# wenet-e2e/wetts

Measured on AMD Instinct MI355X. Metric: audio samples/sec + RTF @22.05 kHz, VITS-Baker, 1/2/4/8 MI355X, higher is better.
Workload: dtype f32

## Files before the change

wetts_amd/csrc/common.h:

```cpp
#pragma once
#include <hip/hip_runtime.h>
#include <stdint.h>
#include <stdio.h>
#include <string>

#include <string.h>

#include "../../include/wetts_hip.h"

namespace wetts {

void set_error(const char* fmt, ...);

#define WETTS_HIP_CHECK(expr)                                                        \
  do {                                                                               \
    hipError_t _e = (expr);                                                          \
    if (_e != hipSuccess) {                                                          \
      ::wetts::set_error("%s failed: %s (%s:%d)", #expr, hipGetErrorString(_e),      \
                         __FILE__, __LINE__);                                        \
      return WETTS_E_HIP;                                                            \
    }                                                                                \
  } while (0)

static inline bool lds_opt_in(const void* kernel, signed char* state) {
// ... 89 lines not shown
  int64_t wn_mask_stride;
  int wn_H, wn_last, wn_first;
};

inline ConvParams conv_io(const float* x, int Cin, int T, float* out, int Cout, int B) {
  ConvParams p;
  memset(&p, 0, sizeof(p));
  p.x = x;
  p.x_bs = (int64_t)Cin * T;
  p.x_cs = T;
  p.Tin = T;
  p.in_rev_base = -1;
  p.in_act = IN_NONE;
  p.in_slope = 0.f;
  p.out = out;
  p.o_bs = (int64_t)Cout * T;
  p.o_cs = T;
  p.Tout = T;
  p.out_act = OUT_NONE;
  p.out_div = 1.f;
  p.B = B;
  return p;
}

struct PackedConv {
  float* wpk = nullptr;
  const float* bias = nullptr;
  int M = 0, Cin = 0, ktaps = 0, dil = 1, pad = 0;
  int up = 0, up_pad = 0;
  int Cout = 0;
  int k_orig = 0;
  int off_lo = 0, span = 0, nchunks = 0;
  int gate_H = 0;
};

int32_t pack_conv_weight(const float* w_dev, const float* bias_dev, int Cout, int Cin, int k,
                         int dil, int pad, int transposed, int up, hipStream_t stream,
                         PackedConv* out, int rev_in = 0, int gate_H = 0);
void free_packed(PackedConv* pc);

int32_t launch_conv(const PackedConv& pc, ConvParams p, hipStream_t stream);
bool pw_gemm_eligible(const PackedConv& pc, const ConvParams& p);
int32_t launch_pw_gemm(const PackedConv& pc, const ConvParams& p, hipStream_t stream, int variant);
int32_t launch_conv_group(const PackedConv* const* pcs, const ConvParams* ps, int n, hipStream_t stream,
                          int* launches = nullptr);

int conv_variant();
void set_conv_variant(int v);
int32_t launch_conv_small(const ConvParams& p, hipStream_t stream, bool* taken);
struct SmallConvScope {
  explicit SmallConvScope(int max_tiles);
  ~SmallConvScope();
  int prev;
};

inline int cdiv(int a, int b) { return (a + b - 1) / b; }
inline int64_t align_up(int64_t v, int64_t a) { return (v + a - 1) / a * a; }

inline int device_cus() {
  static int cus = 0;
  if (cus == 0) {
    int dev = 0, n = 0;
    cus = (hipGetDevice(&dev) == hipSuccess &&
           hipDeviceGetAttribute(&n, hipDeviceAttributeMultiprocessorCount, dev) == hipSuccess && n > 0) ? n : 256;
  }
  return cus;
}

}
```

wetts_amd/csrc/conv_mfma.hip:

```cpp
#include <stdlib.h>

#include "common.h"

namespace wetts {

typedef float f32x16 __attribute__((ext_vector_type(16)));
typedef float f32x4v __attribute__((ext_vector_type(4)));
constexpr int kBufRsrcDword3 = 0x00020000;

__device__ __forceinline__ float lrelu2(float x, float slope) {
  const float m = x * slope;
  float r;
  asm("v_max_f32 %0, %1, %2" : "=v"(r) : "v"(x), "v"(m));
  return r;
}

__global__ void pack_conv_weight_kernel(const float* __restrict__ w, float* __restrict__ out,
                                        int M, int Cin, int Cout, int k, int ktaps, int up,
                                        int transposed, int rev_in, int gate_H, int G, int64_t total) {
  int64_t idx = (int64_t)blockIdx.x * blockDim.x + threadIdx.x;
  if (idx >= total) return;
  int s = (int)(idx & 3);
  int lane = (int)((idx >> 2) & 63);
  int64_t rest = idx >> 8;
// ... 36 lines not shown
    pc->dil = dil;
    pc->pad = pad;
    pc->up = 0;
    pc->up_pad = 0;
  } else {
    pc->M = Cout * up;
    pc->ktaps = cdiv(k, up);
    pc->dil = -1;
    pc->pad = 0;
    pc->up = up;
    pc->up_pad = pad;
  }
  int o0 = -pc->pad, o1 = (pc->ktaps - 1) * pc->dil - pc->pad;
  pc->off_lo = o0 < o1 ? o0 : o1;
  pc->span = (o0 < o1 ? o1 : o0) - pc->off_lo;
  pc->nchunks = cdiv(Cin, kConvCK);
  int G = pc->nchunks * pc->ktaps * 2;
  int mt32 = cdiv(pc->M, 128) * 4;
  int64_t total = (int64_t)mt32 * G * 256;
  WETTS_HIP_CHECK(hipMalloc((void**)&pc->wpk, (total + (int64_t)G * 256) * sizeof(float)));
  WETTS_HIP_CHECK(hipMemsetAsync(pc->wpk + total, 0, (size_t)G * 256 * sizeof(float), stream));
  int threads = 256;
  int64_t blocks = (total + threads - 1) / threads;
  hipLaunchKernelGGL(pack_conv_weight_kernel, dim3((unsigned)blocks), dim3(threads), 0, stream,
                     w_dev, pc->wpk, pc->M, Cin, Cout, k, pc->ktaps, up > 0 ? up : 1, transposed,
                     rev_in, gate_H, G, total);
  WETTS_LAUNCH_CHECK();
  return WETTS_OK;
}

void free_packed(PackedConv* pc) {
  if (pc->wpk) (void)hipFree(pc->wpk);
  pc->wpk = nullptr;
}

constexpr int conv_fixed_stride(int nt) { return ((nt + 132 - 32 + 63) / 64) * 64 + 32; }
constexpr bool conv_has_fixed_stride(int nt) { return nt <= 256; }

template <int MB, int NB, int WM, int WN, int EPI, bool FAST>
__device__ __forceinline__ void conv_mfma_body(const ConvParams& p, int bid) {
  static_assert(WM * WN == 4, "4 waves per block");
  constexpr int CK = kConvCK;
  constexpr int MT = 32 * MB * WM;
  constexpr int NT = 32 * NB * WN;
  constexpr int MAXCI = (NT + 128 + 63) / 64;
  constexpr int RPW = CK / 4;

  extern __shared__ __attribute__((aligned(16))) float smem[];

  const int tid = threadIdx.x;
  const int lane = tid & 63;
  const int wave = __builtin_amdgcn_readfirstlane(tid >> 6);
  const int wm = wave / WN, wn = wave % WN;

  const int ntiles = (p.N + NT - 1) / NT;
  const int mtiles = (p.M + MT - 1) / MT;
  const int ntile = bid % ntiles;
  bid /= ntiles;
  const int mtile = bid % mtiles;
  const int b = bid / mtiles;

  const int n0 = ntile * NT;
  int Tin = p.Tin, Tout = p.Tout, N = p.N;
  if (p.lens) {
    Tin = min((int)p.lens[b] * p.len_mul, p.Tin);
    Tout = p.up > 0 ? Tin * p.up : Tin;
// ... 426 lines not shown
        if (omask) v *= omask[t];
        float* dst = p.out + ob + (int64_t)co * p.o_cs + t;
        if (!pre_res) {
          if (p.res) v += p.res[rb + (int64_t)co * p.r_cs + t];
          if (p.accum) v += *dst;
        }
        if (p.out_div != 1.f) v = mrf_div(v, p.out_div, 1.f / p.out_div, mrf_div_fast(p.out_div));
        *dst = v;
      }
    }
  }
}

template <int MB, int NB, int WM, int WN, int EPI = 0, bool MRF = false, bool FAST = false>
__global__ __launch_bounds__(256) __attribute__((amdgpu_waves_per_eu((MB * NB >= 4 && WN < 4) ? 3 : 1)))
void conv_mfma_kernel(const ConvParams p) {
  conv_mfma_body<MB, NB, WM, WN, EPI, FAST>(p, blockIdx.x);
}

constexpr int kConvGroupMax = 3;
struct ConvGroupParams {
  ConvParams p[kConvGroupMax];
  int first[kConvGroupMax + 1];
  int n;
};
template <int MB, int NB, int WM, int WN, int EPI>
__global__ __launch_bounds__(256) __attribute__((amdgpu_waves_per_eu((MB * NB >= 4 && WN < 4) ? 3 : 1)))
void conv_mfma_group_kernel(const ConvGroupParams gp) {
  const int bid = blockIdx.x;
  int j = 0;
  if (gp.n > 1 && bid >= gp.first[1]) j = 1;
  if (gp.n > 2 && bid >= gp.first[2]) j = 2;
  conv_mfma_body<MB, NB, WM, WN, EPI, true>(gp.p[j], bid - gp.first[j]);
}



static bool conv_fast_ok(const ConvParams& p);

static int g_conv_variant = -1;

int conv_variant() {
  if (g_conv_variant < 0) {
    const char* e = getenv("WETTS_CONV_VARIANT");
    g_conv_variant = e ? atoi(e) : 0;
  }
  return g_conv_variant;
}
void set_conv_variant(int v) { g_conv_variant = v; }

template <int MB, int NB, int WM, int WN>
static int32_t launch_cfg(const ConvParams& p, hipStream_t stream) {
  constexpr int MT = 32 * MB * WM, NT = 32 * NB * WN;
  int ntiles = cdiv(p.N, NT), mtiles = cdiv(p.M, MT);
  int64_t blocks = (int64_t)ntiles * mtiles * p.B;
  if (blocks <= 0) return WETTS_OK;
  WETTS_REQUIRE(blocks < (1ll << 31), "conv grid too large");
  const bool fast = conv_fast_ok(p);
  const size_t lds = (size_t)2 * kConvCK *
                     (fast ? (conv_has_fixed_stride(NT) ? conv_fixed_stride(NT) : ((NT + p.span + 3 + 3) & ~3)) : NT + p.span) *
                     sizeof(float);
  const dim3 grid((unsigned)blocks), blk(256);
  const bool plain = p.up == 0 && p.out_act == OUT_NONE && p.out_mask == nullptr && p.wn_skip == nullptr;
  if (p.out_act == OUT_GATE) {
    if (fast)
      hipLaunchKernelGGL((conv_mfma_kernel<MB, NB, WM, WN, 5, false, true>), grid, blk, lds, stream, p);
// ... 43 lines not shown
  p.ktaps = pc.ktaps;
  p.dil = pc.dil;
  p.pad = pc.pad;
  p.off_lo = pc.off_lo;
  p.span = pc.span;
  p.nchunks = pc.nchunks;
  p.up = pc.up;
  p.up_pad = pc.up_pad;
  p.up_shift = -1;
  for (int q = 0; q < 16; ++q)
    if (pc.up == (1 << q)) p.up_shift = q;
  WETTS_REQUIRE(pc.wpk != nullptr, "conv weight not packed");
  WETTS_REQUIRE((p.out_act == OUT_GATE) == (pc.gate_H > 0), "gate epilogue and interleaved packing go together");
  WETTS_REQUIRE(p.out_act != OUT_GATE || (!p.res && !p.accum && !p.out_mask && p.out_div == 1.f && !p.wn_skip && pc.up == 0),
                "gate epilogue: plain store only");
  if (pc.ktaps == 1 && pc.up == 0 && p.in_mask && p.in_mask == p.out_mask &&
      p.in_mask_stride == p.out_mask_stride && p.out_act == OUT_NONE)
    p.in_mask = nullptr;
  WETTS_REQUIRE(p.span <= 128, "conv receptive field too wide (span %d > 128)", p.span);
  if (p.up > 0) {
    p.N = p.Tin + p.ktaps - 1;
  } else {
    p.N = p.Tout;
  }
  return WETTS_OK;
}

static bool conv_fast_ok(const ConvParams& p) {
  return p.in_mask == nullptr && p.in_rev_base < 0 && (p.Cin % kConvCK) == 0 && (p.x_cs & 3) == 0 &&
         (p.x_bs & 3) == 0 && (p.Tin & 3) == 0 && p.span <= 125 && (reinterpret_cast<uintptr_t>(p.x) & 15) == 0 &&
         ((int64_t)p.Cin * p.x_cs) < (1ll << 29) && (p.lens == nullptr || (p.len_mul & 3) == 0);
}

template <int MB, int NB, int WM, int WN>
static int32_t launch_group_cfg(ConvGroupParams& gp, int max_span, hipStream_t stream) {
  constexpr int MT = 32 * MB * WM, NT = 32 * NB * WN;
  int64_t total = 0;
  for (int j = 0; j < gp.n; ++j) {
    gp.first[j] = (int)total;
    total += (int64_t)cdiv(gp.p[j].N, NT) * cdiv(gp.p[j].M, MT) * gp.p[j].B;
  }
  gp.first[gp.n] = (int)total;
  WETTS_REQUIRE(total > 0 && total < (1ll << 31), "conv group grid size");
  const size_t lds = (size_t)2 * kConvCK * (conv_has_fixed_stride(NT) ? conv_fixed_stride(NT) : ((NT + max_span + 3 + 3) & ~3)) *
                     sizeof(float);
  hipLaunchKernelGGL((conv_mfma_group_kernel<MB, NB, WM, WN, 1>), dim3((unsigned)total), dim3(256), lds, stream, gp);
  WETTS_LAUNCH_CHECK();
  return WETTS_OK;
}

int32_t launch_conv_group(const PackedConv* const* pcs, const ConvParams* ps, int n, hipStream_t stream,
                          int* launches) {
  if (launches) *launches = n;
  if (n <= 0) return WETTS_OK;
  ConvGroupParams gp;
  memset(&gp, 0, sizeof(gp));
  bool ok = n >= 2 && n <= kConvGroupMax && conv_variant() == 0;
  int order[kConvGroupMax] = {0, 1, 2};
  if (ok) {
    for (int a = 0; a < n; ++a)
      for (int b = a + 1; b < n; ++b)
        if (pcs[order[b]]->ktaps > pcs[order[a]]->ktaps) { int t = order[a]; order[a] = order[b]; order[b] = t; }
  }
  int max_span = 0;
  for (int j = 0; j < n && ok; ++j) {
    gp.p[j] = ps[order[j]];
    WETTS_TRY(prepare_conv(*pcs[order[j]], gp.p[j]));
    const ConvParams& q = gp.p[j];
    ok = q.up == 0 && q.out_act == OUT_NONE && q.out_mask == nullptr && q.out_div == 1.f && q.tag && conv_fast_ok(q) &&
         q.M == gp.p[0].M && q.N == gp.p[0].N && q.B == gp.p[0].B && q.Cin == gp.p[0].Cin && q.lens == gp.p[0].lens;
    if (q.span > max_span) max_span = q.span;
  }
  gp.n = n;
  if (ok) {
    const ConvParams& q = gp.p[0];
    const int64_t cols = (int64_t)q.N * q.B;
    auto nblk = [&](int mt, int nt) { return (int64_t)cdiv(q.M, mt) * cdiv(q.N, nt) * q.B; };
    if (q.M >= 128 && cols >= 4096 && nblk(128, 128) >= 384) {
      if (launches) *launches = 1;
      return launch_group_cfg<1, 4, 4, 1>(gp, max_span, stream);
    }
    if (q.M > 32 && q.M < 128 && cols >= 8192 && nblk(64, 256) >= 384) {
      if (launches) *launches = 1;
      return launch_group_cfg<1, 4, 2, 2>(gp, max_span, stream);
    }
  }
  for (int j = 0; j < n; ++j) WETTS_TRY(launch_conv(*pcs[j], ps[j], stream));
  return WETTS_OK;
}

int32_t launch_conv(const PackedConv& pc, ConvParams p, hipStream_t stream) {
  WETTS_TRY(prepare_conv(pc, p));
  if (conv_variant() == 0 && p.lens == nullptr) {
    bool taken = false;
    WETTS_TRY(launch_conv_small(p, stream, &taken));
    if (taken) return WETTS_OK;
  }
  {
    const int v = conv_variant();
    if ((v == 0 || (v >= 7 && v <= 9)) && pw_gemm_eligible(pc, p)) return launch_pw_gemm(pc, p, stream, v);
  }
  const int64_t cols = (int64_t)p.N * p.B;
  switch (conv_variant()) {
    case 2: return launch_cfg<1, 2, 4, 1>(p, stream);
    case 3: return launch_cfg<1, 4, 2, 2>(p, stream);
    case 4: return launch_cfg<1, 2, 2, 2>(p, stream);
    case 5: return launch_cfg<1, 1, 2, 2>(p, stream);
    case 6: return launch_cfg<1, 4, 4, 1>(p, stream);
    default: break;
  }
  auto nblk = [&](int mt, int nt) { return (int64_t)cdiv(p.M, mt) * cdiv(p.N, nt) * p.B; };
  constexpr int64_t kFill = 384;
  if (p.M >= 128 && cols >= 4096) {
    const int64_t n128 = nblk(128, 128);
    const int kCUs = device_cus();
    if (n128 >= 4 * kCUs) return launch_cfg<1, 4, 4, 1>(p, stream);
    auto cost = [&](int64_t blocks, int area, double eff) {
      return (blocks < kCUs ? 4.0 : 1.0) * (double)((blocks + kCUs - 1) / kCUs) * area / eff;
    };
    const double c128 = cost(n128, 128 * 128, 1.18), c64w = cost(nblk(64, 128), 64 * 128, 1.07),
                 c64 = cost(nblk(64, 64), 64 * 64, 1.0);
    if (c128 <= c64w && c128 <= c64) return launch_cfg<1, 4, 4, 1>(p, stream);
    if (c64w <= c64) return launch_cfg<1, 2, 2, 2>(p, stream);
    return launch_cfg<1, 1, 2, 2>(p, stream);
  }
// ... 11 lines not shown
```

wetts_amd/csrc/kernels.hip:

```cpp
#include "kernels.h"

namespace wetts {

static inline dim3 grid1d(int64_t n, int threads) {
  return dim3((unsigned)((n + threads - 1) / threads));
}

__global__ void embed_mask_kernel(const int64_t* __restrict__ ids,
                                  const int64_t* __restrict__ lengths,
                                  const float* __restrict__ emb, int n_vocab, int B, int H, int T,
                                  float scale, float* __restrict__ x_out,
                                  float* __restrict__ mask_out, int32_t* __restrict__ status) {
  int64_t idx = (int64_t)blockIdx.x * blockDim.x + threadIdx.x;
  int64_t total = (int64_t)B * H * T;
  if (idx >= total) return;
  int t = (int)(idx % T);
  int c = (int)((idx / T) % H);
  int b = (int)(idx / ((int64_t)T * H));
  bool valid = (int64_t)t < lengths[b];
  float v = 0.f;
  if (valid) {
    int64_t id = ids[(int64_t)b * T + t];
    if (id < 0 || id >= n_vocab) {
      if (status && c == 0) atomicOr(status, WETTS_STATUS_PHONE_ID_RANGE);
// ... 622 lines not shown
#pragma unroll
        for (int i = 0; i < 10; ++i) win[i] = raw[i] > 0.f ? raw[i] : raw[i] * 0.01f;
#pragma unroll
        for (int j = 0; j < 7; ++j) {
          const float wv = wsh[(c + u) * 7 + j];
#pragma unroll
          for (int o = 0; o < 4; ++o) acc[o] += wv * win[o + j];
        }
      }
    }
  } else
  for (int c = 0; c < C; ++c) {
    const float* xr = xb + (int64_t)c * T;
    float win[4 + 15];
    for (int i = 0; i < 3 + k; ++i) {
      int tt = t0 - pad + i;
      float v = (tt >= 0 && tt < Tb) ? xr[tt] : 0.f;
      win[i] = v > 0.f ? v : v * 0.01f;
    }
    for (int j = 0; j < k; ++j) {
      float wv = wsh[c * k + j];
#pragma unroll
      for (int o = 0; o < 4; ++o) acc[o] += wv * win[o + j];
    }
  }
#pragma unroll
  for (int o = 0; o < 4; ++o)
    if (t0 + o < T) out[(int64_t)b * T + t0 + o] = (t0 + o < Tb) ? tanhf(acc[o]) : 0.f;
}

template <int K>
__global__ __launch_bounds__(256) void conv_post_tanh_small_kernel(const float* __restrict__ x,
                                                                   const float* __restrict__ w, int B,
                                                                   int C, int T, float* __restrict__ out) {
  constexpr int TL = 32, CG = 8, MAXC = 8;
  __shared__ float red[CG][TL + 1];
  const int tl = threadIdx.x % TL, cg = threadIdx.x / TL;
  const int tblocks = (T + TL - 1) / TL;
  const int b = blockIdx.x / tblocks;
  const int t = (blockIdx.x % tblocks) * TL + tl;
  constexpr int pad = (K - 1) / 2;
  const float* xb = x + (int64_t)b * C * T;
  float win[MAXC][K], wv[MAXC][K];
#pragma unroll
  for (int j = 0; j < MAXC; ++j) {
    const int c = cg + CG * j;
    const int cc = c < C ? c : 0;
#pragma unroll
    for (int i = 0; i < K; ++i) {
      const int tt = t - pad + i;
      const bool ok = c < C && tt >= 0 && tt < T;
      win[j][i] = xb[(int64_t)cc * T + (ok ? tt : 0)];
      wv[j][i] = ok ? w[cc * K + i] : 0.f;
    }
  }
  float acc = 0.f;
#pragma unroll
  for (int j = 0; j < MAXC; ++j)
#pragma unroll
    for (int i = 0; i < K; ++i) {
      const float v = win[j][i];
      acc += wv[j][i] * (v > 0.f ? v : v * 0.01f);
    }
  red[cg][tl] = acc;
  __syncthreads();
  if (cg == 0 && t < T) {
    float tot = 0.f;
#pragma unroll
    for (int q = 0; q < CG; ++q) tot += red[q][tl];
    out[(int64_t)b * T + t] = tanhf(tot);
  }
}

int32_t k_conv_post_tanh(const float* x, const float* w, int k, int B, int C, int T, float* out,
                         hipStream_t s, const int64_t* lens, int len_mul) {
  WETTS_REQUIRE(k <= 15, "conv_post kernel size %d unsupported", k);
  int64_t n = (int64_t)B * ((T + 3) / 4);
  if (n == 0) return WETTS_OK;
  if (k == 7 && C <= 64 && n <= 64 * 256 && !lens) {
    hipLaunchKernelGGL(conv_post_tanh_small_kernel<7>, dim3((unsigned)(B * cdiv(T, 32))), dim3(256), 0, s, x, w,
                       B, C, T, out);
    WETTS_LAUNCH_CHECK();
    return WETTS_OK;
  }
  hipLaunchKernelGGL(conv_post_tanh_kernel, grid1d(n, 256), dim3(256), (size_t)C * k * 4, s, x, w,
                     k, B, C, T, out, lens, len_mul);
  WETTS_LAUNCH_CHECK();
  return WETTS_OK;
}

__global__ __launch_bounds__(64) void durations_kernel(const float* __restrict__ logw,
                                                       const float* __restrict__ mask,
                                                       float length_scale, int B, int T,
                                                       float* __restrict__ w_ceil,
                                                       float* __restrict__ cum,
                                                       int64_t* __restrict__ y_lengths,
                                                       int32_t* __restrict__ status) {
  const int b = blockIdx.x, lane = threadIdx.x;
  float carry = 0.f;
  for (int t0 = 0; t0 < T; t0 += 64) {
    int t = t0 + lane;
    float wc = 0.f;
    if (t < T) {
      float w = expf(logw[(int64_t)b * T + t]) * mask[(int64_t)b * T + t] * length_scale;
      wc = ceilf(w);
      w_ceil[(int64_t)b * T + t] = wc;
    }
    float v = wc;
#pragma unroll
    for (int off = 1; off < 64; off <<= 1) {
      float n = __shfl_up(v, off, 64);
      if (lane >= off) v += n;
    }
    v += carry;
// ... 564 lines not shown
```

wetts_amd/csrc/model.hip:

```cpp
#include <stdarg.h>
#include <stdlib.h>
#include <string.h>

#include <map>
#include <string>
#include <vector>

#include "common.h"
#include "conv_bf16.h"
#include "resblock32.h"
#include "qconv_u8.h"
#include "kernels.h"

namespace wetts {

static thread_local char g_err[512] = "";

void set_error(const char* fmt, ...) {
  va_list ap;
  va_start(ap, fmt);
  vsnprintf(g_err, sizeof(g_err), fmt, ap);
  va_end(ap);
}

// ... 366 lines not shown
  int fuse32_maxc = 32;
  int fuse32_kmax = 99;
  int fuse32_kwide = 3;
  int fuse2_maxc = 128;
  int fuse_min_blocks = 128;
  int small_max_tiles = 256;
  int chain_whole_waste_pct = 15;
  int chain_whole_maxc = 64;
  int chain_pair_maxc = 32;
  int chain_pair_kmax = 3;
  int fuse2_waste_pct = 20;
  mutable int flow_precision = 0;
  mutable std::vector<std::vector<PackedConvB>> b_wn_in, b_wn_rs;
  mutable PackedConvB b_post;
  mutable float* b_post_wpad = nullptr;
  mutable PackedQConv q_pre, q_cond, q_post;
  mutable std::vector<std::vector<PackedQConv>> q_c1, q_c2;
  mutable bool q_packed = false;
  mutable int flow_packed_prec = 0, dec_packed_prec = 0;
  mutable std::vector<PackedConvB> b_ups;
  mutable PackedConvB b_pre;
  mutable std::vector<std::vector<PackedConvB>> b_c1, b_c2;
  mutable int32_t* status_word = nullptr;
  mutable uint64_t rng_seed = 0, rng_offset = 0;
  int mrf_streams = 1;
  int mrf_fork_maxc = 1 << 20;
  int stage2_pct = 30;
  int dds_fused = 1;
  int attn_small_max_t = 128;
  int wn_gate = 1;
  int wn_fuse = 1;
  int small_fork = 1;
  int conv_groups = 1;
  hipStream_t aux_stream[WETTS_MAX_RB_KERNELS] = {};
  hipEvent_t ev_fork = nullptr, ev_chain[WETTS_MAX_RB_KERNELS] = {};
  bool fork_ok = false;

  int spec_channels = 0;
  bool post_loaded = false;
  Layout post_layout;
  float* post_blob = nullptr;
  PackedConv pe_pre, pe_proj;
  std::vector<PackedConv> pe_in, pe_rs, fwd_pre;
  const float *pe_cond_w = nullptr, *pe_cond_b = nullptr;

  bool dur_loaded = false;
  Layout dur_layout;
  float* dur_blob = nullptr;
  ConvFlowW dur_cf1;
  std::vector<ConvFlowW> dur_post_cf;
  const float *dur_post_pre_w = nullptr, *dur_post_pre_b = nullptr;
  PackedConv dur_post_proj;
  DDS dur_post_dds;
  const float *dur_qm = nullptr, *dur_qlogs = nullptr;

  const float* T(const std::string& name) const { return tensor(layout, blob, name); }
};

namespace wetts {

struct Bump {
  char* base;
  int64_t cap, off = 0;
  bool ok = true;
  Bump(void* p, int64_t c) : base((char*)p), cap(c) {}
  template <typename T>
// ... 481 lines not shown
  return L.total;
}

int32_t wetts_create(const wetts_config_t* cfg, const float* blob_dev, int64_t blob_numel,
                     void* stream, wetts_model_t** out) {
  WETTS_TRY(validate_config(cfg));
  WETTS_REQUIRE(out != nullptr && blob_dev != nullptr, "null argument");
  hipStream_t s = (hipStream_t)stream;
  wetts_model* m = new wetts_model();
  m->cfg = *cfg;
  build_layout(cfg, m->layout);
  if (blob_numel != m->layout.total) {
    set_error("blob has %lld floats, layout needs %lld", (long long)blob_numel,
              (long long)m->layout.total);
    delete m;
    return WETTS_E_INVALID;
  }
  hipError_t e = hipMalloc((void**)&m->blob, (size_t)blob_numel * sizeof(float));
  if (e != hipSuccess) {
    set_error("hipMalloc(blob) failed: %s", hipGetErrorString(e));
    delete m;
    return WETTS_E_HIP;
  }
  e = hipMemcpyAsync(m->blob, blob_dev, (size_t)blob_numel * sizeof(float),
                     hipMemcpyDeviceToDevice, s);
  int32_t r = (e == hipSuccess) ? build_model(m, s) : WETTS_E_HIP;
  {
    struct Knob { const char* name; int* field; };
    const Knob knobs[] = {
        {"stage2_pct", &m->stage2_pct}, {"dds_fused", &m->dds_fused}, {"wn_fuse", &m->wn_fuse}, {"wn_gate", &m->wn_gate},
        {"fuse2_waste_pct", &m->fuse2_waste_pct}, {"fuse_min_blocks", &m->fuse_min_blocks},
        {"chain_whole_pct", &m->chain_whole_waste_pct}, {"chain_whole_maxc", &m->chain_whole_maxc},
        {"small_max_tiles", &m->small_max_tiles}, {"attn_small_max_t", &m->attn_small_max_t},
    };
    if (const char* env = getenv("WETTS_TUNE")) {
      std::string all(env);
      size_t pos = 0;
      while (pos < all.size()) {
        size_t end = all.find(',', pos);
        if (end == std::string::npos) end = all.size();
        const std::string item = all.substr(pos, end - pos);
        const size_t eq = item.find('=');
        bool known = false;
        if (eq != std::string::npos)
          for (const Knob& k : knobs)
            if (item.compare(0, eq, k.name) == 0 && strlen(k.name) == eq) {
              *k.field = atoi(item.c_str() + eq + 1);
              known = true;
            }
        if (!known && !item.empty()) {
          set_error("WETTS_TUNE: unknown setting '%s'", item.c_str());
          r = WETTS_E_INVALID;
        }
        pos = end + 1;
      }
    }
    if (r == WETTS_OK && !m->wn_gate) {
      for (int f = 0; f < cfg->flow_n_flows && r == WETTS_OK; ++f)
        for (int i = 0; i < cfg->flow_wn_layers && r == WETTS_OK; ++i) {
          free_packed(&m->flows[f].in_layers[i]);
          r = pack(m->layout, m->blob, S("flow.flows.%d.enc.in_layers.%d", flow_key_stride(cfg) * f, i), s,
                   &m->flows[f].in_layers[i]);
        }
    }
    if (m->mrf_streams < 1) m->mrf_streams = 1;
    if (m->mrf_streams > cfg->n_resblock_kernels) m->mrf_streams = cfg->n_resblock_kernels;
    m->fork_ok = hipEventCreateWithFlags(&m->ev_fork, hipEventDisableTiming) == hipSuccess && m->ev_fork;
    for (int j = 0; j < cfg->n_resblock_kernels; ++j) {
      if (hipEventCreateWithFlags(&m->ev_chain[j], hipEventDisableTiming) != hipSuccess || !m->ev_chain[j]) m->fork_ok = false;
      if (j > 0)
        if (hipStreamCreateWithFlags(&m->aux_stream[j], hipStreamNonBlocking) != hipSuccess || !m->aux_stream[j]) m->fork_ok = false;
    }
    (void)hipGetLastError();
  }
  if (r == WETTS_OK) {
    e = hipStreamSynchronize(s);
    if (e != hipSuccess) {
      set_error("weight packing failed: %s", hipGetErrorString(e));
      r = WETTS_E_HIP;
    }
  }
  if (r != WETTS_OK) {
    wetts_destroy(m);
    return r;
  }
  *out = m;
  return WETTS_OK;
}

void wetts_destroy(wetts_model_t* m) {
  if (!m) return;
  free_posterior(m);
  free_duration(m);
  for (PackedConv* pc : m->all_packed) free_packed(pc);
  for (auto& pc : m->b_ups) free_packed_bf16(&pc);
  for (auto& v : m->b_c1) for (auto& pc : v) free_packed_bf16(&pc);
// ... 1223 lines not shown
        p2.r_bs = (int64_t)ch * len;
        p2.r_cs = len;
        p2.accum = accum;
        p2.out_div = odiv;
        p2.tag = 1;
        p2.lens = lens;
        p2.len_mul = spf;
        if (last_d || m->dec_unfused) {
          WETTS_TRY(launch_conv(rb.c2[d], p2, s));
          count(1, 3 + accum);
        } else {
          g2[n2] = &rb.c2[d];
          p2s[n2++] = p2;
        }
      }
      rx[j] = outp[j];
    }
    if (n2 > 0) {
      int nl = 0;
      WETTS_TRY(launch_conv_group(g2, p2s, n2, s, &nl));
      count(nl, 3.0 * n2);
    }
  }
  return WETTS_OK;
}

static int32_t run_hifigan(const wetts_model* m, const float* z, int64_t z_bs, int64_t z_cs,
                           const float* y_mask, int64_t mask_stride, const float* g, int B, int L,
                           float* audio, void* workspace, int64_t workspace_bytes, hipStream_t s,
                           DecTiming* tm, const int64_t* lens = nullptr) {
  const wetts_config_t* c = &m->cfg;
  const int I = c->inter_channels, C0 = c->upsample_initial_channel;
  const int64_t mx = dec_max_elems(c, B, L);
  Bump ws(workspace, workspace_bytes);
  float* bx = ws.take<float>(mx);
  float* bt = ws.take<float>(mx);
  float* bs = ws.take<float>(mx);
  float* chain_buf[WETTS_MAX_RB_KERNELS][3];
  for (int j = 0; j < c->n_resblock_kernels; ++j)
    for (int q = 0; q < 3; ++q) chain_buf[j][q] = ws.take<float>(mx);
  float* cond = ws.take<float>((int64_t)B * C0);
  if (!ws.ok) {
    set_error("hifigan: workspace too small (need %lld bytes)",
              (long long)ws_decoder(c, B, L));
    return WETTS_E_WORKSPACE;
  }
  {
    ConvParams p = conv_io(z, I, L, bx, C0, B);
    p.x_bs = z_bs;
    p.x_cs = z_cs;
    if (y_mask) {
      p.in_mask = y_mask;
      p.in_mask_stride = mask_stride;
    }
    if (has_g(c) && g) {
      WETTS_TRY(k_cond_linear(g, m->dec_cond_w, m->dec_cond_b, B, C0, c->gin_channels, cond, s));
      p.bias_b = cond;
      p.bias_b_stride = C0;
    }
    p.lens = lens;
    p.len_mul = 1;
    WETTS_TRY(launch_conv(m->conv_pre, p, s));
  }
  int ch = C0, len = L;
  int spf = 1;
  float* x = bx;
// ... 981 lines not shown
```

Measured before the change: 52.16 million.

## Add Winograd F(2,3) MFMA conv path for HiFi-GAN resblock convolutions

```diff
diff --git a/wetts_amd/csrc/common.h b/wetts_amd/csrc/common.h
--- a/wetts_amd/csrc/common.h
+++ b/wetts_amd/csrc/common.h
@@ -145,12 +145,19 @@
   int k_orig = 0;
   int off_lo = 0, span = 0, nchunks = 0;
   int gate_H = 0;
+  float* wf23 = nullptr;
 };
 
 int32_t pack_conv_weight(const float* w_dev, const float* bias_dev, int Cout, int Cin, int k,
                          int dil, int pad, int transposed, int up, hipStream_t stream,
                          PackedConv* out, int rev_in = 0, int gate_H = 0);
 void free_packed(PackedConv* pc);
+int32_t pack_conv_f23(const float* w_dev, hipStream_t stream, PackedConv* pc);
+struct ConvF23Scope {
+  explicit ConvF23Scope(int min_tiles);
+  ~ConvF23Scope();
+  int prev;
+};
 
 int32_t launch_conv(const PackedConv& pc, ConvParams p, hipStream_t stream);
 bool pw_gemm_eligible(const PackedConv& pc, const ConvParams& p);
diff --git a/wetts_amd/csrc/conv_mfma.hip b/wetts_amd/csrc/conv_mfma.hip
--- a/wetts_amd/csrc/conv_mfma.hip
+++ b/wetts_amd/csrc/conv_mfma.hip
@@ -92,6 +92,8 @@
 void free_packed(PackedConv* pc) {
   if (pc->wpk) (void)hipFree(pc->wpk);
   pc->wpk = nullptr;
+  if (pc->wf23) (void)hipFree(pc->wf23);
+  pc->wf23 = nullptr;
 }
 
 constexpr int conv_fixed_stride(int nt) { return ((nt + 132 - 32 + 63) / 64) * 64 + 32; }
@@ -584,6 +586,285 @@
   if (gp.n > 1 && bid >= gp.first[1]) j = 1;
   if (gp.n > 2 && bid >= gp.first[2]) j = 2;
   conv_mfma_body<MB, NB, WM, WN, EPI, true>(gp.p[j], bid - gp.first[j]);
+}
+
+constexpr int f23_slots(int kt) { return 4 * (kt / 3) + 2 * (kt % 3); }
+constexpr int f23_quads(int kt) { return (f23_slots(kt) + 3) / 4; }
+constexpr int f23_stride(int wn) { return wn == 1 ? 160 : 224; }
+__host__ __device__ inline int f23_pairs(int n, int d) { const int q = n / (2 * d), r = n - q * 2 * d; return q * d + (r < d ? r : d); }
+
+__global__ void pack_conv_f23_kernel(const float* __restrict__ w, float* __restrict__ out, int M, int Cin, int k,
+                                     int nchunks, int64_t total) {
+  int64_t idx = (int64_t)blockIdx.x * blockDim.x + threadIdx.x;
+  if (idx >= total) return;
+  const int ng = k / 3, S = 4 * ng + 2 * (k % 3), SQ = (S + 3) / 4;
+  const int s = (int)(idx & 3), lane = (int)((idx >> 2) & 63);
+  int64_t rest = idx >> 8;
+  const int quad = (int)(rest % SQ);
+  rest /= SQ;
+  const int ks = (int)(rest & 7);
+  rest >>= 3;
+  const int chunk = (int)(rest % nchunks);
+  const int mt32 = (int)(rest / nchunks);
+  const int slot = quad * 4 + s;
+  const int row = mt32 * 32 + (lane & 31), ci = chunk * kConvCK + ks * 2 + (lane >> 5);
+  float v = 0.f;
+  if (row < M && ci < Cin && slot < S) {
+    const float* wr = w + ((int64_t)row * Cin + ci) * k;
+    if (slot < 4 * ng) {
+      const int g = slot >> 2, q = slot & 3;
+      const double w0 = wr[3 * g], w1 = wr[3 * g + 1], w2 = wr[3 * g + 2];
+      v = q == 0 ? wr[3 * g] : q == 1 ? (float)((w0 + w1 + w2) * 0.5) : q == 2 ? (float)((w0 - w1 + w2) * 0.5) : wr[3 * g + 2];
+    } else {
+      const int l = (slot - 4 * ng) >> 1;
+      v = wr[3 * ng + l];
+      if ((slot - 4 * ng) & 1) v = -v;
+    }
+  }
+  out[idx] = v;
+}
+
+int32_t pack_conv_f23(const float* w_dev, hipStream_t stream, PackedConv* pc) {
+  const int k = pc->ktaps;
+  if (pc->wf23 || pc->up != 0 || pc->gate_H != 0 || pc->dil < 1 || (k != 3 && k != 7 && k != 11) ||
+      pc->pad != (k - 1) / 2 * pc->dil || pc->Cin % kConvCK != 0 || pc->M % 64 != 0 || pc->wpk == nullptr)
+    return WETTS_OK;
+  const int SQ = f23_quads(k);
+  const int64_t total = (int64_t)(pc->M / 32) * pc->nchunks * 8 * SQ * 256, tail = (int64_t)3 * SQ * 256;
+  WETTS_HIP_CHECK(hipMalloc((void**)&pc->wf23, (total + tail) * sizeof(float)));
+  WETTS_HIP_CHECK(hipMemsetAsync(pc->wf23 + total, 0, (size_t)tail * sizeof(float), stream));
+  hipLaunchKernelGGL(pack_conv_f23_kernel, dim3((unsigned)((total + 255) / 256)), dim3(256), 0, stream, w_dev, pc->wf23,
+                     pc->M, pc->Cin, k, pc->nchunks, total);
+  WETTS_LAUNCH_CHECK();
+  return WETTS_OK;
+}
+
+template <int KT, int WM, int WN, int EPI>
+__device__ __forceinline__ void conv_f23_body(const ConvParams& p, int bid) {
+  static_assert(WM * WN == 4, "4 waves per block");
+  static_assert(EPI == 1 || EPI == 2, "plain store or the MRF mean");
+  constexpr int CK = kConvCK, RPW = CK / 4;
+  constexpr int NG = KT / 3, NL = KT % 3, SQ = f23_quads(KT);
+  constexpr int PT = 32 * WN, MT = 32 * WM, W = f23_stride(WN);
+
+  extern __shared__ __attribute__((aligned(16))) float smem[];
+
+  const int tid = threadIdx.x;
+  const int lane = tid & 63;
+  const int wave = __builtin_amdgcn_readfirstlane(tid >> 6);
+  const int wm = wave / WN, wn = wave % WN;
+  const int half = lane >> 5;
+  const int d = p.dil;
+
+  const int ntiles = (f23_pairs(p.N, d) + PT - 1) / PT;
+  const int mtiles = p.M / MT;
+  const int ptile = bid % ntiles;
+  bid /= ntiles;
+  const int mtile = bid % mtiles;
+  const int b = __builtin_amdgcn_readfirstlane(bid / mtiles);
+  const int P0 = ptile * PT;
+  const int n0 = P0 + d * (P0 / d);
+  int Tin = p.Tin;
+  if (p.lens) Tin = min((int)p.lens[b] * p.len_mul, p.Tin);
+  const int N = Tin;
+  if (n0 >= N) return;
+
+  float* buf0 = smem;
+  float* buf1 = smem + CK * W;
+  const float* xb = p.x + (int64_t)b * p.x_bs;
+
+  const int tstart = (n0 + p.off_lo) & ~3;
+  const int sh = (n0 + p.off_lo) & 3;
+  const int W4 = min((2 * PT + 2 * d - 1 + p.span + sh + 3) >> 2, W / 4);
+  const int t0c = tstart < 0 ? 0 : tstart;
+  const int vbase = lane * 16 + (tstart - t0c) * 4;
+  const bool wrq = lane < W4;
+  const bool okq = wrq && tstart + 4 * lane >= 0 && tstart + 4 * lane + 4 <= Tin;
+  __amdgpu_buffer_rsrc_t rsx = __builtin_amdgcn_make_buffer_rsrc(
+      const_cast<float*>(xb), 0, __builtin_amdgcn_readfirstlane(((p.Cin - 1) * (int)p.x_cs + p.Tin) * 4), kBufRsrcDword3);
+  f32x4v stage4[RPW];
+  auto load_chunk = [&](int c) {
+#pragma unroll
+    for (int r = 0; r < RPW; ++r) {
+      const int soff = __builtin_amdgcn_readfirstlane(((c * CK + wave + 4 * r) * (int)p.x_cs + t0c) * 4);
+      stage4[r] = f32x4v{0.f, 0.f, 0.f, 0.f};
+      if (okq) stage4[r] = __builtin_amdgcn_raw_buffer_load_b128(rsx, vbase, soff, 0);
+    }
+  };
+  auto store_chunk = [&](float* buf) {
+    const bool lr = p.in_act == IN_LRELU;
+#pragma unroll
+    for (int r = 0; r < RPW; ++r) {
+      if (wrq) {
+        f32x4v v = stage4[r];
+        if (lr) {
+          v.x = lrelu2(v.x, p.in_slope);
+          v.y = lrelu2(v.y, p.in_slope);
+          v.z = lrelu2(v.z, p.in_slope);
+          v.w = lrelu2(v.w, p.in_slope);
+        }
+        *reinterpret_cast<f32x4v*>(buf + (wave + 4 * r) * W + 4 * lane) = v;
+      }
+    }
+  };
+
+  const int P = P0 + wn * 32 + (lane & 31);
+  const int tb = P + d * (P / d);
+  const bool ok0 = tb < N, ok1 = tb + d < N;
+  const int wrow0 = mtile * MT + wm * 32;
+
+  f32x16 m0, m1, m2, m3;
+  {
+    const char* rbase = p.res ? reinterpret_cast<const char*>(p.res + (int64_t)b * p.r_bs + (int64_t)wrow0 * p.r_cs) : nullptr;
+    const char* pbase = reinterpret_cast<const char*>(p.out + (int64_t)b * p.o_bs + (int64_t)wrow0 * p.o_cs);
+    const unsigned rcs4 = (unsigned)p.r_cs * 4u, ocs4 = (unsigned)p.o_cs * 4u;
+    const unsigned c0 = (unsigned)(ok0 ? tb : n0) * 4u, c1 = (unsigned)(ok1 ? tb + d : n0) * 4u;
+    const unsigned rlane = (unsigned)(4 * half) * rcs4, olane = (unsigned)(4 * half) * ocs4;
+    const float* bp = p.bias ? p.bias + wrow0 + 4 * half : nullptr;
+#pragma unroll
+    for (int r = 0; r < 16; ++r) {
+      m0[r] = 0.f;
+      m3[r] = 0.f;
+    }
+    if (rbase) {
+#pragma unroll
+      for (int r = 0; r < 16; ++r) {
+        const unsigned rr = (unsigned)((r & 3) + 8 * (r >> 2));
+        m0[r] = *reinterpret_cast<const float*>(rbase + (rr * rcs4 + rlane + c0));
+        m3[r] = *reinterpret_cast<const float*>(rbase + (rr * rcs4 + rlane + c1));
+      }
+    }
+    if (p.accum) {
+      float pv[16][2];
+#pragma unroll
+      for (int r = 0; r < 16; ++r) {
+        const unsigned rr = (unsigned)((r & 3) + 8 * (r >> 2));
+        pv[r][0] = *reinterpret_cast<const float*>(pbase + (rr * ocs4 + olane + c0));
+        pv[r][1] = *reinterpret_cast<const float*>(pbase + (rr * ocs4 + olane + c1));
+      }
+      __builtin_amdgcn_sched_barrier(0);
+#pragma unroll
+      for (int r = 0; r < 16; ++r) {
+        m0[r] += pv[r][0];
+        m3[r] += pv[r][1];
+      }
+    }
+#pragma unroll
+    for (int r = 0; r < 16; ++r) {
+      const float bv = bp ? bp[(r & 3) + 8 * (r >> 2)] : 0.f;
+      m0[r] += bv;
+      m3[r] = -(m3[r] + bv);
+      m1[r] = 0.f;
+      m2[r] = 0.f;
+    }
+  }
+
+  constexpr int NS = KT == 11 ? 2 : 4;
+  const float4* abase = reinterpret_cast<const float4*>(p.wpk) +
+                        ((int64_t)(mtile * WM + wm) * p.nchunks * 8 * SQ) * 64 + lane;
+  float4 aset[NS][SQ];
+#pragma unroll
+  for (int i = 0; i < NS - 1; ++i)
+#pragma unroll
+    for (int q = 0; q < SQ; ++q) aset[i][q] = abase[(i * SQ + q) * 64];
+#pragma unroll
+  for (int q = 0; q < SQ; ++q) aset[NS - 1][q] = aset[0][q];
+
+  load_chunk(0);
+  store_chunk(buf0);
+  __syncthreads();
+
+  const int cb = half * W + (tb - n0) + sh;
+  int st = NS - 1;
+  for (int c = 0; c < p.nchunks; ++c) {
+    const float* bl = ((c & 1) ? buf1 : buf0) + cb;
+    const bool more = (c + 1) < p.nchunks;
+    if (more) load_chunk(c + 1);
+    float braw[2][KT + 1];
+#pragma unroll
+    for (int j = 0; j <= KT; ++j) braw[0][j] = bl[j * d];
+#pragma unroll
+    for (int s = 0; s < 8; ++s) {
+#pragma unroll
+      for (int q = 0; q < SQ; ++q) aset[(s + NS - 1) % NS][q] = abase[((int64_t)st * SQ + q) * 64];
+      ++st;
+      if (s < 7) {
+#pragma unroll
+        for (int j = 0; j <= KT; ++j) braw[(s + 1) & 1][j] = bl[2 * (s + 1) * W + j * d];
+      }
+      __builtin_amdgcn_sched_barrier(0);
+      auto A = [&](int slot) {
+        const float4 v = aset[s % NS][slot >> 2];
+        return (slot & 3) == 0 ? v.x : (slot & 3) == 1 ? v.y : (slot & 3) == 2 ? v.z : v.w;
+      };
+      const float* a = braw[s & 1];
+#pragma unroll
+      for (int g = 0; g < NG; ++g) {
+        const float a0 = a[3 * g], a1 = a[3 * g + 1], a2 = a[3 * g + 2], a3 = a[3 * g + 3];
+        const float v0 = a0 - a2, v1 = a1 + a2, v2 = a2 - a1, v3 = a1 - a3;
+        m0 = __builtin_amdgcn_mfma_f32_32x32x2f32(A(4 * g + 0), v0, m0, 0, 0, 0);
+        m1 = __builtin_amdgcn_mfma_f32_32x32x2f32(A(4 * g + 1), v1, m1, 0, 0, 0);
+        m2 = __builtin_amdgcn_mfma_f32_32x32x2f32(A(4 * g + 2), v2, m2, 0, 0, 0);
+        m3 = __builtin_amdgcn_mfma_f32_32x32x2f32(A(4 * g + 3), v3, m3, 0, 0, 0);
+      }
+#pragma unroll
+      for (int l = 0; l < NL; ++l) {
+        m0 = __builtin_amdgcn_mfma_f32_32x32x2f32(A(4 * NG + 2 * l), a[3 * NG + l], m0, 0, 0, 0);
+        m3 = __builtin_amdgcn_mfma_f32_32x32x2f32(A(4 * NG + 2 * l + 1), a[3 * NG + l + 1], m3, 0, 0, 0);
+      }
+    }
+    if (more) store_chunk((c & 1) ? buf0 : buf1);
+    __syncthreads();
+  }
+
+  char* obase = reinterpret_cast<char*>(p.out + (int64_t)b * p.o_bs + (int64_t)wrow0 * p.o_cs);
+  const unsigned ocs4 = (unsigned)p.o_cs * 4u;
+  const unsigned olane = (unsigned)(4 * half) * ocs4 + (unsigned)tb * 4u;
+  const unsigned d4 = (unsigned)d * 4u;
+  const bool vec2 = d == 1 && ((p.o_cs | p.o_bs) & 1) == 0 && (reinterpret_cast<uintptr_t>(p.out) & 7) == 0;
+  auto store_all = [&](auto fin) {
+#pragma unroll
+    for (int r = 0; r < 16; ++r) {
+      const unsigned roff = (unsigned)((r & 3) + 8 * (r >> 2)) * ocs4 + olane;
+      const float y0 = fin((m0[r] + m1[r]) + m2[r]);
+      const float y1 = fin((m1[r] - m2[r]) - m3[r]);
+      if (vec2 && ok1) {
+        float2 v;
+        v.x = y0;
+        v.y = y1;
+        *reinterpret_cast<float2*>(obase + roff) = v;
+      } else {
+        if (ok0) *reinterpret_cast<float*>(obase + roff) = y0;
+        if (ok1) *reinterpret_cast<float*>(obase + (roff + d4)) = y1;
+      }
+    }
+  };
+  if (EPI == 2) {
+    const float dv = p.out_div, dinv = 1.f / p.out_div;
+    if (mrf_div_fast(dv)) store_all([=](float v) { return div_small_const(v, dv, dinv); });
+    else store_all([=](float v) { return v / dv; });
+  } else {
+    store_all([](float v) { return v; });
+  }
+}
+
+template <int KT, int WM, int WN, int EPI>
+__global__ __launch_bounds__(256) __attribute__((amdgpu_waves_per_eu(3)))
+void conv_f23_mrf_kernel(const ConvParams p) {
+  conv_f23_body<KT, WM, WN, EPI>(p, blockIdx.x);
+}
+
+template <int WM, int WN>
+__global__ __launch_bounds__(256) __attribute__((amdgpu_waves_per_eu(3)))
+void conv_f23_mrf_group_kernel(const ConvGroupParams gp) {
+  const int bid = blockIdx.x;
+  int j = 0;
+  if (gp.n > 1 && bid >= gp.first[1]) j = 1;
+  if (gp.n > 2 && bid >= gp.first[2]) j = 2;
+  const int kt = gp.p[j].ktaps;
+  if (kt == 3) conv_f23_body<3, WM, WN, 1>(gp.p[j], bid - gp.first[j]);
+  else if (kt == 7) conv_f23_body<7, WM, WN, 1>(gp.p[j], bid - gp.first[j]);
+  else conv_f23_body<11, WM, WN, 1>(gp.p[j], bid - gp.first[j]);
 }
 
 
@@ -693,6 +974,63 @@
          ((int64_t)p.Cin * p.x_cs) < (1ll << 29) && (p.lens == nullptr || (p.len_mul & 3) == 0);
 }
 
+static thread_local int tls_f23_min_tiles = INT32_MAX;
+ConvF23Scope::ConvF23Scope(int min_tiles) : prev(tls_f23_min_tiles) { tls_f23_min_tiles = min_tiles; }
+ConvF23Scope::~ConvF23Scope() { tls_f23_min_tiles = prev; }
+
+static bool conv_f23_ok(const PackedConv& pc, const ConvParams& p) {
+  const int v = conv_variant();
+  if (v != 0 && v != 10) return false;
+  const int min_tiles = v == 10 ? 0 : tls_f23_min_tiles;
+  if (min_tiles == INT32_MAX || pc.wf23 == nullptr) return false;
+  const int wn = p.M % 128 == 0 ? 1 : 2;
+  const bool ok = p.up == 0 && p.out_act == OUT_NONE && p.out_mask == nullptr && p.wn_skip == nullptr &&
+                  p.bias_b == nullptr && p.tag && p.dil >= 1 && p.Tin == p.Tout && p.N == p.Tout && p.M % 64 == 0 &&
+                  conv_fast_ok(p) && 2 * 32 * wn + 2 * p.dil - 1 + p.span + 6 <= f23_stride(wn) &&
+                  ((int64_t)p.o_cs * 32 + p.Tout) * 4 < (1ll << 32) && ((int64_t)p.r_cs * 32 + p.Tout) * 4 < (1ll << 32);
+  if (!ok) return false;
+  if (min_tiles > 0 && p.M < 128 && p.ktaps == 3) return false;
+  return (int64_t)cdiv(p.M, 64) * cdiv(p.N, 64) * p.B >= min_tiles;
+}
+
+template <int WM, int WN>
+static int32_t launch_f23_cfg(const PackedConv& pc, ConvParams p, hipStream_t stream) {
+  p.wpk = pc.wf23;
+  const int64_t blocks = (int64_t)cdiv(f23_pairs(p.N, p.dil), 32 * WN) * (p.M / (32 * WM)) * p.B;
+  if (blocks <= 0) return WETTS_OK;
+  WETTS_REQUIRE(blocks < (1ll << 31), "conv grid too large");
+  const size_t lds = (size_t)2 * kConvCK * f23_stride(WN) * sizeof(float);
+  const dim3 grid((unsigned)blocks), blk(256);
+#define WETTS_F23_LAUNCH(KT)                                                                                  \
+  if (p.out_div == 1.f) hipLaunchKernelGGL((conv_f23_mrf_kernel<KT, WM, WN, 1>), grid, blk, lds, stream, p); \
+  else hipLaunchKernelGGL((conv_f23_mrf_kernel<KT, WM, WN, 2>), grid, blk, lds, stream, p)
+  if (p.ktaps == 3) { WETTS_F23_LAUNCH(3); }
+  else if (p.ktaps == 7) { WETTS_F23_LAUNCH(7); }
+  else { WETTS_F23_LAUNCH(11); }
+#undef WETTS_F23_LAUNCH
+  WETTS_LAUNCH_CHECK();
+  return WETTS_OK;
+}
+
+static int32_t launch_f23(const PackedConv& pc, const ConvParams& p, hipStream_t stream) {
+  return p.M % 128 == 0 ? launch_f23_cfg<4, 1>(pc, p, stream) : launch_f23_cfg<2, 2>(pc, p, stream);
+}
+
+template <int WM, int WN>
+static int32_t launch_f23_group_cfg(ConvGroupParams& gp, hipStream_t stream) {
+  int64_t total = 0;
+  for (int j = 0; j < gp.n; ++j) {
+    gp.first[j] = (int)total;
+    total += (int64_t)cdiv(f23_pairs(gp.p[j].N, gp.p[j].dil), 32 * WN) * (gp.p[j].M / (32 * WM)) * gp.p[j].B;
+  }
+  gp.first[gp.n] = (int)total;
+  WETTS_REQUIRE(total > 0 && total < (1ll << 31), "conv group grid size");
+  const size_t lds = (size_t)2 * kConvCK * f23_stride(WN) * sizeof(float);
+  hipLaunchKernelGGL((conv_f23_mrf_group_kernel<WM, WN>), dim3((unsigned)total), dim3(256), lds, stream, gp);
+  WETTS_LAUNCH_CHECK();
+  return WETTS_OK;
+}
+
 template <int MB, int NB, int WM, int WN>
 static int32_t launch_group_cfg(ConvGroupParams& gp, int max_span, hipStream_t stream) {
   constexpr int MT = 32 * MB * WM, NT = 32 * NB * WN;
@@ -716,6 +1054,47 @@
   if (n <= 0) return WETTS_OK;
   ConvGroupParams gp;
   memset(&gp, 0, sizeof(gp));
+  if (n <= kConvGroupMax) {
+    int fi[kConvGroupMax], ri[kConvGroupMax], nf = 0, nr = 0;
+    for (int j = 0; j < n; ++j) {
+      ConvParams q = ps[j];
+      WETTS_TRY(prepare_conv(*pcs[j], q));
+      if (conv_f23_ok(*pcs[j], q)) fi[nf++] = j; else ri[nr++] = j;
+    }
+    if (nf > 0) {
+      for (int a = 0; a < nf; ++a)
+        for (int b = a + 1; b < nf; ++b)
+          if (pcs[fi[b]]->ktaps > pcs[fi[a]]->ktaps) { int t = fi[a]; fi[a] = fi[b]; fi[b] = t; }
+      bool same = nf >= 2;
+      for (int j = 0; j < nf; ++j) {
+        gp.p[j] = ps[fi[j]];
+        WETTS_TRY(prepare_conv(*pcs[fi[j]], gp.p[j]));
+        gp.p[j].wpk = pcs[fi[j]]->wf23;
+        const ConvParams& q = gp.p[j];
+        same = same && q.out_div == 1.f && q.M == gp.p[0].M && q.N == gp.p[0].N && q.B == gp.p[0].B &&
+               q.Cin == gp.p[0].Cin && q.lens == gp.p[0].lens;
+      }
+      gp.n = nf;
+      int nl = nf;
+      if (same) {
+        nl = 1;
+        WETTS_TRY(gp.p[0].M % 128 == 0 ? (launch_f23_group_cfg<4, 1>(gp, stream)) : (launch_f23_group_cfg<2, 2>(gp, stream)));
+      } else {
+        for (int j = 0; j < nf; ++j) WETTS_TRY(launch_f23(*pcs[fi[j]], gp.p[j], stream));
+      }
+      if (nr > 0) {
+        const PackedConv* rp[kConvGroupMax];
+        ConvParams rps[kConvGroupMax];
+        for (int j = 0; j < nr; ++j) { rp[j] = pcs[ri[j]]; rps[j] = ps[ri[j]]; }
+        int rl = 0;
+        WETTS_TRY(launch_conv_group(rp, rps, nr, stream, &rl));
+        nl += rl;
+      }
+      if (launches) *launches = nl;
+      return WETTS_OK;
+    }
+    memset(&gp, 0, sizeof(gp));
+  }
   bool ok = n >= 2 && n <= kConvGroupMax && conv_variant() == 0;
   int order[kConvGroupMax] = {0, 1, 2};
   if (ok) {
@@ -752,6 +1131,7 @@
 
 int32_t launch_conv(const PackedConv& pc, ConvParams p, hipStream_t stream) {
   WETTS_TRY(prepare_conv(pc, p));
+  if (conv_f23_ok(pc, p)) return launch_f23(pc, p, stream);
   if (conv_variant() == 0 && p.lens == nullptr) {
     bool taken = false;
     WETTS_TRY(launch_conv_small(p, stream, &taken));
diff --git a/wetts_amd/csrc/kernels.hip b/wetts_amd/csrc/kernels.hip
--- a/wetts_amd/csrc/kernels.hip
+++ b/wetts_amd/csrc/kernels.hip
@@ -678,7 +678,8 @@
 template <int K>
 __global__ __launch_bounds__(256) void conv_post_tanh_small_kernel(const float* __restrict__ x,
                                                                    const float* __restrict__ w, int B,
-                                                                   int C, int T, float* __restrict__ out) {
+                                                                   int C, int T, float* __restrict__ out,
+                                                                   const int64_t* __restrict__ lens, int len_mul) {
   constexpr int TL = 32, CG = 8, MAXC = 8;
   __shared__ float red[CG][TL + 1];
   const int tl = threadIdx.x % TL, cg = threadIdx.x / TL;
@@ -687,6 +688,7 @@
   const int t = (blockIdx.x % tblocks) * TL + tl;
   constexpr int pad = (K - 1) / 2;
   const float* xb = x + (int64_t)b * C * T;
+  const int Tb = lens ? min((int)lens[b] * len_mul, T) : T;
   float win[MAXC][K], wv[MAXC][K];
 #pragma unroll
   for (int j = 0; j < MAXC; ++j) {
@@ -695,7 +697,7 @@
 #pragma unroll
     for (int i = 0; i < K; ++i) {
       const int tt = t - pad + i;
-      const bool ok = c < C && tt >= 0 && tt < T;
+      const bool ok = c < C && tt >= 0 && tt < Tb;
       win[j][i] = xb[(int64_t)cc * T + (ok ? tt : 0)];
       wv[j][i] = ok ? w[cc * K + i] : 0.f;
     }
@@ -714,7 +716,7 @@
     float tot = 0.f;
 #pragma unroll
     for (int q = 0; q < CG; ++q) tot += red[q][tl];
-    out[(int64_t)b * T + t] = tanhf(tot);
+    out[(int64_t)b * T + t] = t < Tb ? tanhf(tot) : 0.f;
   }
 }
 
@@ -723,9 +725,9 @@
   WETTS_REQUIRE(k <= 15, "conv_post kernel size %d unsupported", k);
   int64_t n = (int64_t)B * ((T + 3) / 4);
   if (n == 0) return WETTS_OK;
-  if (k == 7 && C <= 64 && n <= 64 * 256 && !lens) {
+  if (k == 7 && C <= 64 && n <= 64 * 256) {
     hipLaunchKernelGGL(conv_post_tanh_small_kernel<7>, dim3((unsigned)(B * cdiv(T, 32))), dim3(256), 0, s, x, w,
-                       B, C, T, out);
+                       B, C, T, out, lens, len_mul);
     WETTS_LAUNCH_CHECK();
     return WETTS_OK;
   }
diff --git a/wetts_amd/csrc/model.hip b/wetts_amd/csrc/model.hip
--- a/wetts_amd/csrc/model.hip
+++ b/wetts_amd/csrc/model.hip
@@ -422,6 +422,7 @@
   int wn_fuse = 1;
   int small_fork = 1;
   int conv_groups = 1;
+  int conv_f23_min_tiles = 4096;
   hipStream_t aux_stream[WETTS_MAX_RB_KERNELS] = {};
   hipEvent_t ev_fork = nullptr, ev_chain[WETTS_MAX_RB_KERNELS] = {};
   bool fork_ok = false;
@@ -969,6 +970,7 @@
         {"fuse2_waste_pct", &m->fuse2_waste_pct}, {"fuse_min_blocks", &m->fuse_min_blocks},
         {"chain_whole_pct", &m->chain_whole_waste_pct}, {"chain_whole_maxc", &m->chain_whole_maxc},
         {"small_max_tiles", &m->small_max_tiles}, {"attn_small_max_t", &m->attn_small_max_t},
+        {"conv_f23_min_tiles", &m->conv_f23_min_tiles},
     };
     if (const char* env = getenv("WETTS_TUNE")) {
       std::string all(env);
@@ -999,6 +1001,14 @@
           r = pack(m->layout, m->blob, S("flow.flows.%d.enc.in_layers.%d", flow_key_stride(cfg) * f, i), s,
                    &m->flows[f].in_layers[i]);
         }
+    }
+    if (r == WETTS_OK && m->conv_f23_min_tiles != INT32_MAX && cfg->vocoder_type != 1) {
+      for (const GenConv& g : hifigan_convs(cfg)) {
+        if (r != WETTS_OK || (g.kind != GenConv::C1 && g.kind != GenConv::C2)) continue;
+        ConvRef cr;
+        r = find_conv(m->layout, m->blob, g.prefix, &cr);
+        if (r == WETTS_OK) r = pack_conv_f23(cr.w, s, g.kind == GenConv::C1 ? &m->rbs[g.n].c1[g.d] : &m->rbs[g.n].c2[g.d]);
+      }
     }
     if (m->mrf_streams < 1) m->mrf_streams = 1;
     if (m->mrf_streams > cfg->n_resblock_kernels) m->mrf_streams = cfg->n_resblock_kernels;
@@ -2288,6 +2298,7 @@
   const wetts_config_t* c = &m->cfg;
   const int I = c->inter_channels, C0 = c->upsample_initial_channel;
   const int64_t mx = dec_max_elems(c, B, L);
+  ConvF23Scope f23_scope(m->conv_f23_min_tiles);
   Bump ws(workspace, workspace_bytes);
   float* bx = ws.take<float>(mx);
   float* bt = ws.take<float>(mx);
```

After: 57.53 million, median of 6. 1.1x the previous value.
